# DIAGNijmegen/prostateMR_3D-CAD-csPCa

Hardware: AMD Instinct MI355X
Metric: train-step volumes/sec (whole job), M1 (20,160,160,3) (higher is better)
Workload: dtype bf16; 1 GPU; C3 M1 full hierarchical-probabilistic dense_skip+deep_supervision latents (3,2,1,0) (20,160,160,3); batch_per_gpu=2, global_batch=2, params=67254246, parallelism=dp1, hip_graph=True

## Files before the change

prostatemr_3d-cad-cspca_amd/csrc/conv_mfma.h:

```cpp
#pragma once
#include "common.h"
#include "gather.h"
#include "cdna4.h"

#define MF_MAX_TAPS 27
#define MF_MAX_CLASSES 8

struct MfmaP {
    const void* src[M1_MAX_SRC];
    int srcC[M1_MAX_SRC];
    int srcSeg[M1_MAX_SRC];
    int nsrc, CC, spt;
    int ID, IH, IW;
    void* out;
    int OC, OCn;
    int nout;
    void* outs[M1_MAX_SRC]; int outC[M1_MAX_SRC]; int outOff[M1_MAX_SRC + 1]; int outAcc[M1_MAX_SRC];
    int OD, OH, OW, N;
    const void* wp;
    const float* bias;
    const float* bias2; int bias_split;
    int mode, sd, sh, sw, pd, ph, pw;
    int nclasses;
    int cls_ntaps[MF_MAX_CLASSES], cls_first[MF_MAX_CLASSES], cls_kpad[MF_MAX_CLASSES];
    long long cls_woff[MF_MAX_CLASSES];
    signed char tdd[MF_MAX_TAPS], tdh[MF_MAX_TAPS], tdw[MF_MAX_TAPS];
    int tap_pk[MF_MAX_TAPS];
    int accumulate;
    int ksplit;
    float* acc32;
    long long slab_elems;
    int aligned;
    int korder;
    const void* ib_x;
    const float* ib_stats; const float* ib_gamma; const float* ib_beta; float ib_slope;
    int tps;
    float* stat_partial;
    int stat_tiles;
};

struct OutRef { void* base; int C, col, acc; };
__device__ __forceinline__ OutRef m1_out_ref(const MfmaP& p, int oc) {
    if (p.nout == 0) return OutRef{p.out, p.OC, oc, p.accumulate};
    int m = 0;
    while (m + 1 < p.nout && oc >= p.outOff[m + 1]) ++m;
    return OutRef{p.outs[m], p.outC[m], oc - p.outOff[m], p.outAcc[m]};
}

__device__ __forceinline__ float m1_bias_at(const MfmaP& p, int oc) {
    if (p.bias_split > 0 && oc >= p.bias_split) return p.bias2 ? p.bias2[oc - p.bias_split] : 0.f;
    return p.bias ? p.bias[oc] : 0.f;
}

template <typename T> struct MT;
template <> struct MT<bf16_t> { static constexpr int SEG = 8; };
template <> struct MT<float> { static constexpr int SEG = 4; };


bool m1_halo_conv_supported(const MfmaP& mp, int OCpad);
int m1_halo_conv_stat_parts(const MfmaP& mp, int OCpad);
int m1_halo_conv(const MfmaP& mp, int OCpad, hipStream_t st);

bool m1_pw_conv_supported(const MfmaP& mp, int OCpad, int BN);
int m1_pw_conv_stat_parts(const MfmaP& mp, int OCpad, int BN);
int m1_pw_conv(const MfmaP& mp, int OCpad, int BN, hipStream_t st);
```

prostatemr_3d-cad-cspca_amd/csrc/conv_mfma.hip:

```cpp
#include "common.h"
#include "gather.h"
#include "reduce.h"

#include "conv_mfma.h"
#include "conv_t3.h"
#include <stdlib.h>

template <typename T>
__device__ __forceinline__ uint4 load_partial_seg(const T* p, int n) {
    constexpr int SEG = MT<T>::SEG;
    union { uint4 v; T e[SEG]; } u;
    u.v = make_uint4(0, 0, 0, 0);
#pragma unroll
    for (int k = 0; k < SEG; ++k) if (k < n) u.e[k] = p[k];
    return u.v;
}

__device__ __forceinline__ unsigned lds_addr_of(const void* p) { return (unsigned)(unsigned long long)(lptr_t)p; }

template <typename T, int BM, int BN, int WM, int WN, int KC, bool GLDS, int KG = 1>
__global__ void __launch_bounds__(WM * WN * 64 * KG) conv_mfma_kernel(MfmaP p) {
#if defined(__HIP_DEVICE_COMPILE__)
    constexpr int NTHR = WM * WN * 64, NW = WM * WN;
    static_assert(KG == 1 || GLDS, "K groups: LDS-DMA path only");
    constexpr int SEG = MT<T>::SEG;
    constexpr int TM = BM / WM / 16, TN = BN / WN / 16;
    constexpr int A_BYTES = BM * 64, B_BYTES = BN * 64;
    constexpr int A_LD = BM * 4 / NTHR;
    constexpr int B_LD = (BN * 4 + NTHR - 1) / NTHR;
    static_assert((NW == 4 || NW == 8 || NW == 16) && (BM * 4) % NTHR == 0 && BN % 16 == 0, "tile config");

    extern __shared__ __attribute__((aligned(16))) unsigned char smem[];
    int4* rowinfo = reinterpret_cast<int4*>(smem);
    int* outrow = reinterpret_cast<int*>(rowinfo + BM);
    const T** s_src = reinterpret_cast<const T**>(outrow + BM);
    int* s_srcC = reinterpret_cast<int*>(s_src + M1_MAX_SRC);
    int* s_srcSeg = s_srcC + M1_MAX_SRC;
    int* s_tap = s_srcSeg + M1_MAX_SRC;
    int* s_tdl = s_tap + MF_MAX_TAPS;
    constexpr int TBL_BYTES = (BM * 20 + M1_MAX_SRC * 16 + 2 * MF_MAX_TAPS * 4 + 15) / 16 * 16;
    const int kg = KG > 1 ? __builtin_amdgcn_readfirstlane((int)threadIdx.x / NTHR) : 0;
    const int tid = KG > 1 ? (int)threadIdx.x - kg * NTHR : (int)threadIdx.x, lane = tid & 63, wave = tid >> 6;
    constexpr int GROUP_BYTES = 2 * KC * (A_BYTES + B_BYTES);
    unsigned char* A_s = smem + TBL_BYTES + kg * GROUP_BYTES;
    unsigned char* B_s = A_s + 2 * KC * A_BYTES;

    const int wm = wave / WN, wn = wave % WN;
    const int cls = blockIdx.y / p.ksplit, ksp = (blockIdx.y % p.ksplit) * KG + kg;
    const int oc0 = blockIdx.z * BN;

    int pdc = 0, phc = 0, pwc = 0, QD = p.OD, QH = p.OH, QW = p.OW;
    if (p.mode == 1) {
        pwc = cls % p.sw; phc = (cls / p.sw) % p.sh; pdc = cls / (p.sw * p.sh);
        QD = p.OD > pdc ? (p.OD - pdc + p.sd - 1) / p.sd : 0;
        QH = p.OH > phc ? (p.OH - phc + p.sh - 1) / p.sh : 0;
        QW = p.OW > pwc ? (p.OW - pwc + p.sw - 1) / p.sw : 0;
    }
    const long long QV = (long long)QD * QH * QW, Mtot = QV * p.N;
    const long long tile = (long long)(blockIdx.x & 7) * (gridDim.x >> 3) + (blockIdx.x >> 3);
    long long m0 = tile * BM, m_end = Mtot;
    if (p.tps > 0) {
        if (tile >= (long long)p.tps * p.N) return;
        const long long tn = tile / p.tps;
        m0 = tn * QV + (tile - tn * p.tps) * BM; m_end = (tn + 1) * QV;
    }
    if (m0 >= Mtot) return;

    for (int r = tid; r < BM; r += NTHR) {
        const long long m = m0 + r;
        int4 ri = make_int4(-1, 0, 0, 0); int orow = -1;
        if (m < m_end) {
            int n, qw, qh, qd;
            if (Mtot < (1ll << 31)) {
                const unsigned mm = (unsigned)m, qv = (unsigned)QV;
                n = (int)(mm / qv); const unsigned lin = mm - (unsigned)n * qv;
                const unsigned t1 = lin / (unsigned)QW; qw = (int)(lin - t1 * (unsigned)QW);
                qd = (int)(t1 / (unsigned)QH); qh = (int)(t1 - (unsigned)qd * (unsigned)QH);
            } else {
                n = (int)(m / QV); long long lin = m % QV;
                qw = (int)(lin % QW); lin /= QW; qh = (int)(lin % QH); qd = (int)(lin / QH);
            }
            if (p.mode == 0) {
                ri = make_int4(n, qd * p.sd - p.pd, qh * p.sh - p.ph, qw * p.sw - p.pw);
                orow = (int)m;
            } else {
                ri = make_int4(n, qd, qh, qw);
                orow = (int)((((long long)n * p.OD + qd * p.sd + pdc) * p.OH + qh * p.sh + phc) * p.OW + qw * p.sw + pwc);
            }
        }
        rowinfo[r] = ri; outrow[r] = orow;
    }
    if (tid < M1_MAX_SRC) { s_src[tid] = (const T*)p.src[tid]; s_srcC[tid] = p.srcC[tid]; s_srcSeg[tid] = p.srcSeg[tid]; }
    const int ntaps = p.cls_ntaps[cls], tfirst = p.cls_first[cls];
    if (tid < ntaps) {
        const int t = tfirst + tid;
        s_tap[tid] = ((int)p.tdd[t] & 0xff) | (((int)p.tdh[t] & 0xff) << 8) | (((int)p.tdw[t] & 0xff) << 16);
        s_tdl[tid] = ((int)p.tdd[t] * p.IH + (int)p.tdh[t]) * p.IW + (int)p.tdw[t];
    }
    __syncthreads();

    const int spt = p.spt;
    const int nseg = ntaps * spt;
    const int nchunks_all = (nseg + 3) >> 2;
    const int cps = (nchunks_all + p.ksplit * KG - 1) / (p.ksplit * KG);
    const int c_beg = ksp * cps;
    const int nchunks = (c_beg + cps <= nchunks_all ? cps : nchunks_all - c_beg);
    const int kpad = p.cls_kpad[cls];
    const T* wp = (const T*)p.wp + p.cls_woff[cls];

    f32x4_t acc[TM][TN];
#pragma unroll
    for (int i = 0; i < TM; ++i)
#pragma unroll
        for (int j = 0; j < TN; ++j) acc[i][j] = (f32x4_t){0.f, 0.f, 0.f, 0.f};

    uint4 ra[GLDS ? 1 : KC][GLDS ? 1 : A_LD], rb[GLDS ? 1 : KC][GLDS ? 1 : B_LD];
    const int lrow = tid >> 2;
    const int lseg = GLDS ? ((tid & 3) ^ ((-(tid >> 4)) & 3)) : (tid & 3);
    const int wave_u = __builtin_amdgcn_readfirstlane(wave);

    int st_tap = 0, st_s = 0, st_c = 0;
    const T* st_ptr[A_LD];
    auto st_set_tap = [&]() {
        const int tp = s_tap[st_tap];
        const int dd = (signed char)(tp & 0xff), dh = (signed char)((tp >> 8) & 0xff), dw = (signed char)((tp >> 16) & 0xff);
#pragma unroll
        for (int i = 0; i < A_LD; ++i) {
            const int4 ri = rowinfo[lrow + (NTHR / 4) * i];
            const int id = ri.y + dd, ih = ri.z + dh, iw = ri.w + dw;
            st_ptr[i] = nullptr;
            if (ri.x >= 0 && id >= 0 && id < p.ID && ih >= 0 && ih < p.IH && iw >= 0 && iw < p.IW) {
                const long long vox = (((long long)ri.x * p.ID + id) * p.IH + ih) * p.IW + iw;
                st_ptr[i] = s_src[st_s] + vox * s_srcC[st_s] + lseg * SEG;
            }
        }
    };
    constexpr unsigned OOB = 0x80000000u;
    unsigned b_vo[B_LD];
    unsigned rmask[A_LD]; int rvox[A_LD], rbyte[A_LD];
    int tap_db = 0;
    __amdgpu_buffer_rsrc_t rs_a = __builtin_amdgcn_make_buffer_rsrc((void*)p.src[0], 0, 0, 0x00020000);
    auto glds_set_member = [&]() {
        const int sC = __builtin_amdgcn_readfirstlane(s_srcC[st_s]);
#pragma unroll
        for (int i = 0; i < A_LD; ++i) rbyte[i] = (rvox[i] * sC + lseg * SEG) * (int)sizeof(T);
        rs_a = __builtin_amdgcn_make_buffer_rsrc((void*)p.src[__builtin_amdgcn_readfirstlane(st_s)], 0, 0x7fffffff, 0x00020000);
    };
    auto glds_set_tap = [&]() {
        tap_db = __builtin_amdgcn_readfirstlane(s_tdl[st_tap]) * __builtin_amdgcn_readfirstlane(s_srcC[st_s]) * (int)sizeof(T);
    };
    if constexpr (GLDS) {
        int4 ris[A_LD];
#pragma unroll
        for (int i = 0; i < A_LD; ++i) { ris[i] = rowinfo[lrow + (NTHR / 4) * i]; rmask[i] = 0; }
#pragma unroll 9
        for (int t = 0; t < ntaps; ++t) {
            const int tp = s_tap[t];
            const int dd = (signed char)(tp & 0xff), dh = (signed char)((tp >> 8) & 0xff), dw = (signed char)((tp >> 16) & 0xff);
#pragma unroll
            for (int i = 0; i < A_LD; ++i) {
                const bool ok = ris[i].x >= 0 && (unsigned)(ris[i].y + dd) < (unsigned)p.ID && (unsigned)(ris[i].z + dh) < (unsigned)p.IH &&
                                (unsigned)(ris[i].w + dw) < (unsigned)p.IW;
                rmask[i] |= (ok ? 1u : 0u) << t;
            }
        }
#pragma unroll
        for (int i = 0; i < A_LD; ++i) rvox[i] = ((ris[i].x * p.ID + ris[i].y) * p.IH + ris[i].z) * p.IW + ris[i].w;
    }
    if constexpr (GLDS) {
#pragma unroll
        for (int i = 0; i < B_LD; ++i) {
            const int e = tid + NTHR * i;
            b_vo[i] = (unsigned)(((oc0 + (e >> 2)) * kpad + lseg * SEG) * (int)sizeof(T));
        }
    }
    if (p.aligned && nchunks > 0) {
        const int cpt = spt >> 2;
        int c;
        if (p.korder == 2) { const int cg = c_beg / (2 * ntaps), rem = c_beg - cg * 2 * ntaps; st_tap = rem >> 1; c = (cg * 2 + (rem & 1)) * 4 * SEG; }
        else if (p.korder) { const int cg = c_beg / ntaps; st_tap = c_beg - cg * ntaps; c = cg * 4 * SEG; }
        else { st_tap = c_beg / cpt; c = (c_beg - st_tap * cpt) * 4 * SEG; }
        while (c >= s_srcC[st_s]) { c -= s_srcC[st_s]; ++st_s; }
        st_c = c;
        if constexpr (GLDS) { glds_set_member(); glds_set_tap(); } else st_set_tap();
    }

    auto prefetch_stage = [&](int sg) {
#pragma unroll
        for (int kc = 0; kc < KC; ++kc) {
            const int rel = sg * KC + kc;
            const int chunk = c_beg + rel;
            const bool live = rel < nchunks;
#pragma unroll
            for (int i = 0; i < B_LD; ++i) {
                const int e = tid + NTHR * i;
                uint4 v = make_uint4(0, 0, 0, 0);
                if (live && e < BN * 4)
                    v = *reinterpret_cast<const uint4*>(wp + (long long)(oc0 + (e >> 2)) * kpad + (long long)(chunk * 4 + (e & 3)) * SEG);
                rb[kc][i] = v;
            }
            if (!live) {
#pragma unroll
                for (int i = 0; i < A_LD; ++i) ra[kc][i] = make_uint4(0, 0, 0, 0);
            } else if (p.aligned) {
#pragma unroll
                for (int i = 0; i < A_LD; ++i)
                    ra[kc][i] = st_ptr[i] ? *reinterpret_cast<const uint4*>(st_ptr[i] + st_c) : make_uint4(0, 0, 0, 0);
                st_c += 4 * SEG;
                if (st_c >= s_srcC[st_s]) {
                    st_c = 0;
                    if (++st_s == p.nsrc) { st_s = 0; ++st_tap; }
                    if (st_tap < ntaps) st_set_tap();
                }
            } else {
                const int kseg = chunk * 4 + lseg;
                const T* sp = nullptr; int sC = 0, coff = 0, dd = 0, dh = 0, dw = 0;
                const bool kvalid = kseg < nseg;
                if (kvalid) {
                    const int tap_i = kseg / spt;
                    int cs = kseg - tap_i * spt, s = 0;
                    while (cs >= s_srcSeg[s]) { cs -= s_srcSeg[s]; ++s; }
                    sp = s_src[s]; sC = s_srcC[s]; coff = cs * SEG;
                    const int tp = s_tap[tap_i];
                    dd = (signed char)(tp & 0xff); dh = (signed char)((tp >> 8) & 0xff); dw = (signed char)((tp >> 16) & 0xff);
                }
#pragma unroll
                for (int i = 0; i < A_LD; ++i) {
                    const int4 ri = rowinfo[lrow + (NTHR / 4) * i];
                    uint4 v = make_uint4(0, 0, 0, 0);
                    const int id = ri.y + dd, ih = ri.z + dh, iw = ri.w + dw;
                    if (kvalid && coff < sC && ri.x >= 0 && id >= 0 && id < p.ID && ih >= 0 && ih < p.IH && iw >= 0 && iw < p.IW) {
                        const long long vox = (((long long)ri.x * p.ID + id) * p.IH + ih) * p.IW + iw;
                        if (sC % SEG == 0) v = *reinterpret_cast<const uint4*>(sp + vox * sC + coff);
                        else v = load_partial_seg<T>(sp + vox * sC + coff, sC - coff < SEG ? sC - coff : SEG);
                    }
                    ra[kc][i] = v;
                }
            }
        }
    };
    const __amdgpu_buffer_rsrc_t rs_b = __builtin_amdgcn_make_buffer_rsrc((void*)wp, 0, 0x7fffffff, 0x00020000);
    const __amdgpu_buffer_rsrc_t rs_0 = __builtin_amdgcn_make_buffer_rsrc((void*)wp, 0, 0, 0x00020000);
    auto issue_chunk = [&](int kc, int buf, int chunk, const __amdgpu_buffer_rsrc_t ra, const __amdgpu_buffer_rsrc_t rb) {
#pragma unroll
        for (int i = 0; i < B_LD; ++i)
            if ((NW * (i + 1)) * 64 <= BN * 4 || (wave_u + NW * i) * 64 < BN * 4)
                __builtin_amdgcn_raw_ptr_buffer_load_lds(rb, (lptr_t)(B_s + (buf * KC + kc) * B_BYTES + (wave_u + NW * i) * 1024), 16,
                                                         b_vo[i], chunk * 64, 0, 0);
#pragma unroll
        for (int i = 0; i < A_LD; ++i) {
            const unsigned vo = ((rmask[i] >> st_tap) & 1u) ? (unsigned)(rbyte[i] + tap_db) : OOB;
            __builtin_amdgcn_raw_ptr_buffer_load_lds(ra, (lptr_t)(A_s + (buf * KC + kc) * A_BYTES + (wave_u + NW * i) * 1024), 16,
                                                     vo, st_c * (int)sizeof(T), 0, 0);
        }
    };
    auto advance_chunk = [&]() {
        if (p.korder == 2) {
            if (((st_c / (4 * SEG)) & 1) == 0) st_c += 4 * SEG;
            else {
                st_c -= 4 * SEG;
                if (++st_tap == ntaps) {
                    st_tap = 0; st_c += 8 * SEG;
                    if (st_c >= s_srcC[st_s]) { st_c = 0; if (++st_s < p.nsrc) glds_set_member(); }
                }
                if (st_s < p.nsrc) glds_set_tap();
            }
        } else if (p.korder) {
            if (++st_tap == ntaps) {
                st_tap = 0; st_c += 4 * SEG;
                if (st_c >= s_srcC[st_s]) { st_c = 0; if (++st_s < p.nsrc) glds_set_member(); }
            }
            if (st_s < p.nsrc) glds_set_tap();
        } else {
            st_c += 4 * SEG;
            if (st_c >= s_srcC[st_s]) {
                st_c = 0;
                if (++st_s == p.nsrc) { st_s = 0; ++st_tap; }
                if (st_tap < ntaps) { glds_set_member(); glds_set_tap(); }
            }
        }
    };
    auto issue = [&](int sg, int buf) {
        const int rel0 = sg * KC;
        if (rel0 + KC <= nchunks) {
#pragma unroll
            for (int kc = 0; kc < KC; ++kc) { issue_chunk(kc, buf, c_beg + rel0 + kc, rs_a, rs_b); advance_chunk(); }
        } else {
#pragma unroll
            for (int kc = 0; kc < KC; ++kc) {
                const bool live = rel0 + kc < nchunks;
                issue_chunk(kc, buf, c_beg + rel0 + kc, live ? rs_a : rs_0, live ? rs_b : rs_0);
                if (live) advance_chunk();
            }
        }
    };
    auto stage = [&](int buf) {
#pragma unroll
        for (int kc = 0; kc < KC; ++kc) {
#pragma unroll
            for (int i = 0; i < A_LD; ++i) {
                const int row = lrow + (NTHR / 4) * i;
                *reinterpret_cast<uint4*>(A_s + (buf * KC + kc) * A_BYTES + row * 64 + m1_swz64(row, lseg) * 16) = ra[kc][i];
            }
#pragma unroll
            for (int i = 0; i < B_LD; ++i) {
                const int e = tid + NTHR * i;
                if (e < BN * 4) {
                    const int row = e >> 2;
                    *reinterpret_cast<uint4*>(B_s + (buf * KC + kc) * B_BYTES + row * 64 + m1_swz64(row, e & 3) * 16) = rb[kc][i];
                }
            }
        }
    };

    const int fr = lane & 15, fs = lane >> 4;
    const unsigned a_rd = lds_addr_of(A_s) + (wm * (BM / WM) + fr) * 64 + m1_swz64(fr, fs) * 16;
    const unsigned b_rd = lds_addr_of(B_s) + (wn * (BN / WN) + fr) * 64 + m1_swz64(fr, fs) * 16;
    const int nstages = KG > 1 ? (cps + KC - 1) / KC : (nchunks + KC - 1) / KC;
    if (nstages > 0) {
        if constexpr (GLDS) issue(0, 0);
        else { prefetch_stage(0); stage(0); }
    }
    __syncthreads();
    for (int it = 0; it < nstages; ++it) {
        const int buf = it & 1;
        if (it + 1 < nstages) { if constexpr (GLDS) issue(it + 1, buf ^ 1); else prefetch_stage(it + 1); }
        if constexpr (GLDS) {
            u32x4_t af[KC][TM], bfr[KC][TN];
            auto rd = [&](int kc) {
#pragma unroll
                for (int i = 0; i < TM; ++i) af[kc][i] = m1_lds_read128(a_rd + (buf * KC + kc) * A_BYTES + i * 1024);
#pragma unroll
                for (int j = 0; j < TN; ++j) bfr[kc][j] = m1_lds_read128(b_rd + (buf * KC + kc) * B_BYTES + j * 1024);
            };
            rd(0);
#pragma unroll
            for (int kc = 0; kc < KC; ++kc) {
                m1_lds_wait(af[kc][0]);
#pragma unroll
                for (int i = 1; i < TM; ++i) m1_lds_tie(af[kc][i]);
#pragma unroll
                for (int j = 0; j < TN; ++j) m1_lds_tie(bfr[kc][j]);
                if (kc + 1 < KC) rd(kc + 1);
                __builtin_amdgcn_sched_barrier(0);
#pragma unroll
                for (int i = 0; i < TM; ++i)
#pragma unroll
                    for (int j = 0; j < TN; ++j) {
                        if constexpr (sizeof(T) == 2) {
                            acc[i][j] = __builtin_amdgcn_mfma_f32_16x16x32_bf16(__builtin_bit_cast(bf16x8_t, af[kc][i]),
                                                                                __builtin_bit_cast(bf16x8_t, bfr[kc][j]), acc[i][j], 0, 0, 0);
                        } else {
#pragma unroll
                            for (int q = 0; q < 4; ++q)
                                acc[i][j] = __builtin_amdgcn_mfma_f32_16x16x4f32(__uint_as_float(af[kc][i][q]), __uint_as_float(bfr[kc][j][q]), acc[i][j], 0, 0, 0);
                        }
                    }
                if (kc + 1 < KC) __builtin_amdgcn_sched_barrier(0);
            }
        } else {
#pragma unroll
        for (int kc = 0; kc < KC; ++kc) {
            uint4 af[TM], bfr[TN];
#pragma unroll
            for (int i = 0; i < TM; ++i) {
                const int row = wm * (BM / WM) + i * 16 + fr;
                af[i] = *reinterpret_cast<const uint4*>(A_s + (buf * KC + kc) * A_BYTES + row * 64 + m1_swz64(row, fs) * 16);
            }
#pragma unroll
            for (int j = 0; j < TN; ++j) {
                const int row = wn * (BN / WN) + j * 16 + fr;
                bfr[j] = *reinterpret_cast<const uint4*>(B_s + (buf * KC + kc) * B_BYTES + row * 64 + m1_swz64(row, fs) * 16);
            }
#pragma unroll
            for (int i = 0; i < TM; ++i)
#pragma unroll
                for (int j = 0; j < TN; ++j) {
                    if constexpr (sizeof(T) == 2) {
                        acc[i][j] = __builtin_amdgcn_mfma_f32_16x16x32_bf16(__builtin_bit_cast(bf16x8_t, af[i]),
                                                                            __builtin_bit_cast(bf16x8_t, bfr[j]), acc[i][j], 0, 0, 0);
                    } else {
                        acc[i][j] = __builtin_amdgcn_mfma_f32_16x16x4f32(__uint_as_float(af[i].x), __uint_as_float(bfr[j].x), acc[i][j], 0, 0, 0);
                        acc[i][j] = __builtin_amdgcn_mfma_f32_16x16x4f32(__uint_as_float(af[i].y), __uint_as_float(bfr[j].y), acc[i][j], 0, 0, 0);
                        acc[i][j] = __builtin_amdgcn_mfma_f32_16x16x4f32(__uint_as_float(af[i].z), __uint_as_float(bfr[j].z), acc[i][j], 0, 0, 0);
                        acc[i][j] = __builtin_amdgcn_mfma_f32_16x16x4f32(__uint_as_float(af[i].w), __uint_as_float(bfr[j].w), acc[i][j], 0, 0, 0);
                    }
                }
        }
        }
        if constexpr (!GLDS) { if (it + 1 < nstages) stage(buf ^ 1); }
        __syncthreads();
    }

    if constexpr (KG > 1) {
        float* const xr = reinterpret_cast<float*>(smem + TBL_BYTES);
        if (kg > 0) {
            float* dst = xr + ((size_t)(kg - 1) * NTHR + tid) * (TM * TN * 4);
#pragma unroll
            for (int i = 0; i < TM; ++i)
#pragma unroll
                for (int j = 0; j < TN; ++j) *reinterpret_cast<f32x4_t*>(dst + (i * TN + j) * 4) = acc[i][j];
        }
        __syncthreads();
        if (kg > 0) return;
#pragma unroll
        for (int g = 1; g < KG; ++g) {
            const float* src = xr + ((size_t)(g - 1) * NTHR + tid) * (TM * TN * 4);
#pragma unroll
            for (int i = 0; i < TM; ++i)
#pragma unroll
                for (int j = 0; j < TN; ++j) acc[i][j] += *reinterpret_cast<const f32x4_t*>(src + (i * TN + j) * 4);
        }
        __syncthreads();
    }
    if (p.ksplit > 1) {
        float* slab = p.acc32 + (long long)ksp * p.slab_elems;
#pragma unroll
        for (int i = 0; i < TM; ++i)
#pragma unroll
            for (int j = 0; j < TN; ++j) {
                const int oc = oc0 + wn * (BN / WN) + j * 16 + fr;
#pragma unroll
                for (int r = 0; r < 4; ++r) {
                    const int orow = outrow[wm * (BM / WM) + i * 16 + fs * 4 + r];
                    if (orow >= 0 && oc < p.OCn) slab[(long long)orow * p.OC + oc] = acc[i][j][r];
                }
            }
        return;
    }
    constexpr int CP = BN + SEG;
    T* C_s = reinterpret_cast<T*>(A_s);
#pragma unroll
    for (int i = 0; i < TM; ++i)
#pragma unroll
        for (int j = 0; j < TN; ++j) {
            const int col = wn * (BN / WN) + j * 16 + fr;
            const float bv = (oc0 + col < p.OCn) ? m1_bias_at(p, oc0 + col) : 0.f;
#pragma unroll
            for (int r = 0; r < 4; ++r) {
                const int row = wm * (BM / WM) + i * 16 + fs * 4 + r;
                Act<T>::st(C_s + row * CP + col, acc[i][j][r] + bv);
            }
        }
    __syncthreads();
    if (p.stat_partial) {
        constexpr int EPI_BYTES = (int)((BM * CP * sizeof(T) + 15) / 16 * 16), PIPE_BYTES = 2 * KC * (A_BYTES + B_BYTES) * KG;
        float* red = reinterpret_cast<float*>(A_s + (PIPE_BYTES > EPI_BYTES ? PIPE_BYTES : EPI_BYTES));
        constexpr int G = NTHR / BN;
        const int col = tid % BN, rg = tid / BN;
        float s = 0.f, ss = 0.f;
        if (p.ib_x) {
            const int oc = oc0 + col < p.OCn ? oc0 + col : 0, n = (int)(m0 / QV);
            const float mean = p.ib_stats[((long long)n * p.OC + oc) * 2], rstd = p.ib_stats[((long long)n * p.OC + oc) * 2 + 1];
            const float gm = p.ib_gamma[oc], bt = p.ib_beta[oc];
            const T* xb = (const T*)p.ib_x + oc;
            constexpr int RPT = (BM + G - 1) / G;
            if constexpr (RPT > 32) {
                for (int row = rg; row < BM; row += G) {
                    const int orow = outrow[row];
                    if (orow >= 0) {
                        const float xh = (Act<T>::ld(xb + (long long)orow * p.OC) - mean) * rstd;
                        const float dy = Act<T>::ld(C_s + row * CP + col) * lrelu_g(gm * xh + bt, p.ib_slope);
                        s += dy; ss += dy * xh;
                    }
                }
            } else {
            float xv[RPT];
#pragma unroll
            for (int i = 0; i < RPT; ++i) {
                const int row = rg + i * G;
                const int orow = row < BM ? outrow[row] : -1;
                xv[i] = orow >= 0 ? Act<T>::ld(xb + (long long)orow * p.OC) : 0.f;
            }
#pragma unroll
            for (int i = 0; i < RPT; ++i) {
                const int row = rg + i * G;
                if (row < BM && outrow[row] >= 0) {
                    const float xh = (xv[i] - mean) * rstd;
                    const float dy = Act<T>::ld(C_s + row * CP + col) * lrelu_g(gm * xh + bt, p.ib_slope);
                    s += dy; ss += dy * xh;
                }
            }
            }
        } else
        for (int row = rg; row < BM; row += G) {
            if (outrow[row] >= 0) { const float v = Act<T>::ld(C_s + row * CP + col); s += v; ss += v * v; }
        }
        red[tid * 2] = s; red[tid * 2 + 1] = ss;
        __syncthreads();
        if (rg == 0 && oc0 + col < p.OCn) {
            for (int q = 1; q < G; ++q) { s += red[(q * BN + col) * 2]; ss += red[(q * BN + col) * 2 + 1]; }
            float* dst = p.stat_partial + ((tile * p.OC) + oc0 + col) * 2;
            dst[0] = s; dst[1] = ss;
        }
    }
    constexpr int SPR = BN / SEG;
    for (int e = tid; e < BM * SPR; e += NTHR) {
        const int row = e / SPR, cs = e % SPR;
        const int orow = outrow[row];
        const int oc = oc0 + cs * SEG;
        if (orow < 0 || oc >= p.OCn) continue;
        const OutRef o = m1_out_ref(p, oc);
        if (!o.base) continue;
        uint4 v = *reinterpret_cast<const uint4*>(C_s + row * CP + cs * SEG);
        T* dst = (T*)o.base + (long long)orow * o.C + o.col;
        if (o.C % SEG != 0 || (p.nout == 0 && oc + SEG > p.OCn)) {
            union { uint4 q; T e[SEG]; } ve; ve.q = v;
#pragma unroll
            for (int k = 0; k < SEG; ++k) {
                if (oc + k < p.OCn) {
                    float a = Act<T>::ld(&ve.e[k]);
                    if (o.acc) a += Act<T>::ld(dst + k);
                    Act<T>::st(dst + k, a);
                }
            }
            continue;
        }
        if (o.acc) {
            float a[SEG], b[SEG];
            VecIO<T, SEG>::ld(reinterpret_cast<const T*>(&v), a);
            VecIO<T, SEG>::ld(dst, b);
#pragma unroll
            for (int k = 0; k < SEG; ++k) a[k] += b[k];
            VecIO<T, SEG>::st(dst, a);
        } else {
            *reinterpret_cast<uint4*>(dst) = v;
        }
    }
#endif
}

template <typename T, int BM, int BN, int KC, int NTHR, int KG = 1>
static constexpr size_t mfma_smem_bytes() {
    size_t tbl = (BM * 20 + M1_MAX_SRC * 16 + 2 * MF_MAX_TAPS * 4 + 15) / 16 * 16;
    size_t pipe = (size_t)KC * (2 * BM * 64 + 2 * BN * 64) * KG;
    size_t epi = ((size_t)BM * (BN + MT<T>::SEG) * sizeof(T) + 15) / 16 * 16;
    return tbl + (pipe > epi ? pipe : epi) + NTHR * 2 * sizeof(float);
}

struct PackP {
    const float* w; long long wST, wSC, wSO; int oc_off, cc_off, OCn, OCpad, CC;
    const float* w2; long long w2ST, w2SC, w2SO; int oc_split, c_split;
    int nsrc, spt, SEG; int srcC[M1_MAX_SRC], srcSeg[M1_MAX_SRC];
    int nclasses; int cls_ntaps[MF_MAX_CLASSES], cls_first[MF_MAX_CLASSES], cls_kpad[MF_MAX_CLASSES];
    long long cls_woff[MF_MAX_CLASSES];
    unsigned char wtap[MF_MAX_TAPS];
    int korder;
};
__device__ __forceinline__ bool pack_seg_pos(const PackP& p, int cls, int kseg, int* nvalid, int* wtap, int* chan) {
    int tap_i, seg;
    if (p.korder == 2) {
        const int chunk = kseg >> 2, nt = p.cls_ntaps[cls], cg = chunk / (2 * nt), rem = chunk - cg * 2 * nt;
        tap_i = rem >> 1; seg = (cg * 2 + (rem & 1)) * 4 + (kseg & 3);
    } else if (p.korder) {
        const int chunk = kseg >> 2, nt = p.cls_ntaps[cls], cg = chunk / nt;
        tap_i = chunk - cg * nt; seg = cg * 4 + (kseg & 3);
    } else { tap_i = kseg / p.spt; seg = kseg - tap_i * p.spt; }
    int c = 0, s = 0;
    while (s < p.nsrc && seg >= p.srcSeg[s]) { seg -= p.srcSeg[s]; c += p.srcC[s]; ++s; }
    if (s >= p.nsrc || tap_i >= p.cls_ntaps[cls]) { *nvalid = 0; return false; }
    const int rem = p.srcC[s] - seg * p.SEG;
    *nvalid = rem < p.SEG ? rem : p.SEG;
    *chan = c + seg * p.SEG;
    *wtap = p.wtap[p.cls_first[cls] + tap_i];
    return true;
}
#define M1_PACK_JOB_BYTES 512
#define M1_PACK_MAGIC 0x4d315031u
struct PackJob { PackP p; void* out; int dtype; unsigned magic; };
static_assert(sizeof(PackJob) <= M1_PACK_JOB_BYTES, "pack job record");

template <typename T>
__device__ __forceinline__ void pack_class_elems(const PackP& p, int cls, T* __restrict__ out, long long first, long long stride) {
    constexpr int SEG = MT<T>::SEG;
    const int kpad = p.cls_kpad[cls], nks = kpad / SEG;
    const bool oc_fast = p.wSO == 1;
    const int ocg = p.OCpad >> 4, ksg = (nks + 3) >> 2;
    const long long tot = oc_fast ? (long long)ocg * ksg * 64 : (long long)p.OCpad * nks;
    for (long long u = first; u < tot; u += stride) {
        int oc, kseg;
        if (oc_fast) {
            const long long grp = u >> 6; const int l = (int)(u & 63);
            oc = (int)(grp % ocg) * 16 + (l & 15); kseg = (int)(grp / ocg) * 4 + (l >> 4);
            if (kseg >= nks) continue;
        } else { oc = (int)(u / nks); kseg = (int)(u % nks); }
        int nvalid, wtap = 0, c = 0;
        pack_seg_pos(p, cls, kseg, &nvalid, &wtap, &c);
// ... 103 lines not shown
    }
    __device__ void vec(int n, long long v, int c0, float (*acc)[kVec]) const {
        const long long row = (long long)n * V + v, i = row * OC + c0;
        float a[kVec];
#pragma unroll
        for (int e = 0; e < kVec; ++e) {
            const int oc = c0 + e;
            a[e] = (bias_split > 0 && oc >= bias_split) ? (bias2 ? bias2[oc - bias_split] : 0.f) : (bias ? bias[oc] : 0.f);
        }
        for (int k = 0; k < ksplit; ++k) {
            const float* sp = acc32 + (long long)k * slab + i;
#pragma unroll
            for (int q = 0; q < kVec; q += 4) {
                const float4 t = *reinterpret_cast<const float4*>(sp + q);
                a[q] += t.x; a[q + 1] += t.y; a[q + 2] += t.z; a[q + 3] += t.w;
            }
        }
        T* dst = out + i;
        if (fo.nout > 0) {
            int m = 0;
            while (m + 1 < fo.nout && c0 >= fo.outOff[m + 1]) ++m;
            dst = (T*)fo.outs[m] + row * fo.outC[m] + (c0 - fo.outOff[m]);
        }
        VecIO<T, kVec>::st(dst, a);
        float xv[kVec];
        if (ib_x) VecIO<T, kVec>::ld(ib_x + i, xv);
#pragma unroll
        for (int e = 0; e < kVec; ++e) {
            float r = a[e];
            if constexpr (sizeof(T) == 2) r = bf2f(f2bf(r));
            if (ib_x) {
                const int c = c0 + e;
                const float xh = (xv[e] - ib_stats[((long long)n * OC + c) * 2]) * ib_stats[((long long)n * OC + c) * 2 + 1];
                const float dy = r * lrelu_g(ib_gamma[c] * xh + ib_beta[c], ib_slope);
                acc[0][e] += dy; acc[1][e] += dy * xh;
            } else { acc[0][e] += r; acc[1][e] += r * r; }
        }
    }
};

static inline int seg_of(int dtype) { return dtype == M1_BF16 ? 8 : 4; }
static inline int pick_bn(int ocn) { return ocn > 64 ? 128 : (ocn > 32 ? 64 : (ocn > 16 ? 32 : 16)); }
struct Plan { int BN, BM, ksplit; };
static inline bool want_bn160(const GatherSpec& g) {
    int en = M1_CFG("M1_BN160", 1);
    return en && g.dtype == M1_BF16 && g.w2 && g.oc_split > 0 && g.mode == 0 && g.OC % 160 == 0 && g.OC <= 320;
}
static inline Plan make_plan(int ocn, long long maxM, int ncls, int min_nchunks, bool bn160 = false) {
    Plan pl; pl.BN = bn160 ? 160 : pick_bn(ocn);
    const int ntile = (ocn + pl.BN - 1) / pl.BN;
    pl.BM = (bn160 || cdiv_ll(maxM, 128) * ncls * ntile >= 256) ? 128 : 64;
    const long long blocks = cdiv_ll(maxM, pl.BM) * ncls * ntile;
    pl.ksplit = 1;
    {
        int t128 = M1_CFG("M1_PLAN128", 768);
        const long long b128 = cdiv_ll(maxM, 128) * ncls * ntile;
        if (t128 > 0 && pl.BN == 128 && b128 >= 100 && b128 < t128 && min_nchunks >= 200) {
            pl.BM = 128;
            long long want = cdiv_ll(t128, b128), cap = min_nchunks / 64;
            pl.ksplit = (int)(want < cap ? want : cap);
            if (pl.ksplit < 1) pl.ksplit = 1;
            return pl;
        }
    }
    if (blocks < 256 && min_nchunks >= 16) {
        long long want = cdiv_ll(512, blocks), cap = min_nchunks / 8;
        pl.ksplit = (int)(want < cap ? want : cap);
        if (pl.ksplit < 1) pl.ksplit = 1;
        if (pl.ksplit > 32) pl.ksplit = 32;
    }
    return pl;
}
static inline long long spec_maxM(const GatherSpec& g) {
    if (g.mode == 0) return (long long)g.N * g.OD * g.OH * g.OW;
    return (long long)g.N * ((g.OD + g.sd - 1) / g.sd) * ((g.OH + g.sh - 1) / g.sh) * ((g.OW + g.sw - 1) / g.sw);
}
static inline int spec_ncls(const GatherSpec& g) { return g.mode == 1 ? g.sd * g.sh * g.sw : 1; }

bool m1_mfma_supported(const GatherSpec& g) {
    if (g.kd * g.kh * g.kw > MF_MAX_TAPS) return false;
    if (g.mode == 1 && g.sd * g.sh * g.sw > MF_MAX_CLASSES) return false;
    return true;
}

static inline int spec_spt(const GatherSpec& g, int SEG) {
    int s = 0; for (int i = 0; i < g.nsrc; ++i) s += (g.srcC[i] + SEG - 1) / SEG; return s;
}
static void build_classes(const GatherSpec& g, int CC, int SEG, int OCpad, MfmaP* mp, PackP* pp, long long* total_elems) {
    const int ncls = g.mode == 1 ? g.sd * g.sh * g.sw : 1;
    int t = 0; long long woff = 0;
    for (int c = 0; c < ncls; ++c) {
        const int pwc = g.mode == 1 ? c % g.sw : 0, phc = g.mode == 1 ? (c / g.sw) % g.sh : 0, pdc = g.mode == 1 ? c / (g.sw * g.sh) : 0;
        const int first = t;
        for (int a = 0; a < g.kd; ++a) {
            int od;
            if (g.mode == 0) od = a - 0; else { int v = pdc + g.pd - a; if (v % g.sd) continue; od = v / g.sd; }
            for (int b = 0; b < g.kh; ++b) {
                int oh;
                if (g.mode == 0) oh = b; else { int v = phc + g.ph - b; if (v % g.sh) continue; oh = v / g.sh; }
                for (int e = 0; e < g.kw; ++e) {
                    int ow;
                    if (g.mode == 0) ow = e; else { int v = pwc + g.pw - e; if (v % g.sw) continue; ow = v / g.sw; }
                    if (mp) { mp->tdd[t] = (signed char)od; mp->tdh[t] = (signed char)oh; mp->tdw[t] = (signed char)ow; }
                    if (pp) pp->wtap[t] = (unsigned char)((a * g.kh + b) * g.kw + e);
                    ++t;
                }
            }
        }
        const int nt = t - first;
        const int nseg = nt * spec_spt(g, SEG);
        const int kpad = ((nseg + 3) / 4) * 4 * SEG;
        if (mp) { mp->cls_ntaps[c] = nt; mp->cls_first[c] = first; mp->cls_kpad[c] = kpad; mp->cls_woff[c] = woff; }
        if (pp) { pp->cls_ntaps[c] = nt; pp->cls_first[c] = first; pp->cls_kpad[c] = kpad; pp->cls_woff[c] = woff; }
        woff += (long long)OCpad * kpad;
    }
    if (mp) mp->nclasses = ncls;
    if (pp) pp->nclasses = ncls;
    *total_elems = woff;
}

static inline int min_class_chunks(const GatherSpec& g, int CC, int SEG) {
    MfmaP tmp{}; long long tot = 0;
    build_classes(g, CC, SEG, 16, &tmp, nullptr, &tot);
    int mn = 1 << 30;
    for (int c = 0; c < tmp.nclasses; ++c) { int n = tmp.cls_kpad[c] / (4 * SEG); if (n < mn) mn = n; }
    return mn;
}
static inline size_t out_elems(const GatherSpec& g) { return (size_t)g.N * g.OD * g.OH * g.OW * g.OC; }

size_t m1_mfma_ws_bytes(const GatherSpec& g) {
    const int SEG = seg_of(g.dtype);
    int CC = 0; for (int i = 0; i < g.nsrc; ++i) CC += g.srcC[i];
    size_t best = 0;
    const bool maybe160 = g.dtype == M1_BF16 && g.mode == 0 && g.OC % 160 == 0 && g.OC <= 320;
    int t3bn = 0, t3ks = 1;
    const bool t3 = m1_ct3_plan(g, &t3bn, &t3ks);
    for (int v = 0; v < 3; ++v) {
        if ((v == 1 && !maybe160) || (v == 2 && !t3)) continue;
        Plan pl = make_plan(g.OC, spec_maxM(g), spec_ncls(g), min_class_chunks(g, CC, SEG), v == 1);
        if (v == 2) { pl.BN = t3bn; pl.BM = 256; pl.ksplit = t3ks; }
        const int BN = pl.BN, OCpad = (g.OC + BN - 1) / BN * BN;
        long long tot = 0;
        build_classes(g, CC, SEG, OCpad, nullptr, nullptr, &tot);
        size_t bytes = ((size_t)tot * (g.dtype == M1_BF16 ? 2 : 4) + 255) / 256 * 256;
        if (pl.ksplit > 1) bytes += out_elems(g) * sizeof(float) * pl.ksplit;
        if (bytes > best) best = bytes;
    }
    return best + 256 + M1_PACK_JOB_BYTES;
}

template <typename T, int BM, int BN, int WM, int WN, int KC>
static int launch_cfg_kc(const MfmaP& mp, long long maxM, int OCpad, hipStream_t st) {
    dim3 grid((unsigned)(cdiv_ll(cdiv_ll(maxM, BM), 8) * 8), mp.nclasses * mp.ksplit, OCpad / BN);
    const size_t smem = mfma_smem_bytes<T, BM, BN, KC, WM * WN * 64>();
    auto kern = mp.aligned ? conv_mfma_kernel<T, BM, BN, WM, WN, KC, true> : conv_mfma_kernel<T, BM, BN, WM, WN, KC, false>;
    if (smem > 48 * 1024 && m1_allow_dynamic_lds((const void*)kern, (int)smem) != M1_OK) return M1_ERR_LAUNCH;
    m1_note_kernel("conv_mfma:%dx%d:w%d:ks%d", BM, BN, WM * WN, mp.ksplit);
    hipLaunchKernelGGL(kern, grid, dim3(WM * WN * 64), smem, st, mp);
    return m1_check_launch();
}

template <typename T, int BM, int BN, int WM, int WN, int KG>
static int launch_cfg_kg(const MfmaP& mp, long long maxM, int OCpad, hipStream_t st) {
    constexpr size_t smem = mfma_smem_bytes<T, BM, BN, 2, WM * WN * 64, KG>();
    if constexpr (sizeof(T) != 2 || smem > 160 * 1024 - 256 || WM * WN * 64 * KG > 1024) return M1_ERR_UNSUPPORTED;
    else {
        dim3 grid((unsigned)(cdiv_ll(cdiv_ll(maxM, BM), 8) * 8), mp.nclasses * mp.ksplit, OCpad / BN);
        if (m1_allow_dynamic_lds((const void*)conv_mfma_kernel<T, BM, BN, WM, WN, 2, true, KG>, (int)smem) != M1_OK) return M1_ERR_LAUNCH;
        m1_note_kernel("conv_mfma:%dx%d:w%d:ks%d:kg%d", BM, BN, WM * WN, mp.ksplit, KG);
        hipLaunchKernelGGL((conv_mfma_kernel<T, BM, BN, WM, WN, 2, true, KG>), grid, dim3(WM * WN * 64 * KG), smem, st, mp);
        return m1_check_launch();
    }
}
static inline int mfma_kg_max(int BM, int BN, int nthr) {
    const int group = 2 * 2 * (BM + BN) * 64;
    int k = (150 * 1024) / group; if (k > 1024 / nthr) k = 1024 / nthr; if (k > 4) k = 4;
    return k >= 2 ? k : 0;
}

template <typename T, int BM, int BN, int WM, int WN>
static int launch_cfg(const MfmaP& mp, long long maxM, int OCpad, hipStream_t st, int kg = 1) {
    if (kg == 2) return launch_cfg_kg<T, BM, BN, WM, WN, 2>(mp, maxM, OCpad, st);
    if (kg == 3) return launch_cfg_kg<T, BM, BN, WM, WN, 3>(mp, maxM, OCpad, st);
    if (kg == 4) return launch_cfg_kg<T, BM, BN, WM, WN, 4>(mp, maxM, OCpad, st);
    int minchunks = 1 << 30;
    for (int c = 0; c < mp.nclasses; ++c) { const int n = mp.cls_kpad[c] / (4 * MT<T>::SEG) / mp.ksplit; if (n < minchunks) minchunks = n; }
    return minchunks >= 6 ? launch_cfg_kc<T, BM, BN, WM, WN, 2>(mp, maxM, OCpad, st)
                          : launch_cfg_kc<T, BM, BN, WM, WN, 1>(mp, maxM, OCpad, st);
}

template <typename T>
static int run_mfma(const GatherSpec& g, void* ws, int ws_packed, hipStream_t st) {
    constexpr int SEG = MT<T>::SEG;
    MfmaP mp{}; PackP pp{};
    int CC = 0;
    for (int i = 0; i < M1_MAX_SRC; ++i) {
        mp.src[i] = i < g.nsrc ? g.src[i] : nullptr; mp.srcC[i] = i < g.nsrc ? g.srcC[i] : (1 << 30);
        mp.srcSeg[i] = i < g.nsrc ? (g.srcC[i] + SEG - 1) / SEG : (1 << 30);
        pp.srcC[i] = i < g.nsrc ? g.srcC[i] : 0; pp.srcSeg[i] = i < g.nsrc ? (g.srcC[i] + SEG - 1) / SEG : 0;
        if (i < g.nsrc) CC += g.srcC[i];
    }
    mp.nsrc = g.nsrc; mp.CC = CC; mp.spt = spec_spt(g, SEG);
    pp.nsrc = g.nsrc; pp.spt = mp.spt; pp.SEG = SEG; mp.ID = g.ID; mp.IH = g.IH; mp.IW = g.IW; mp.out = g.out; mp.OC = g.OC; mp.OCn = g.OC;
    void* panel = reinterpret_cast<unsigned char*>(ws) + M1_PACK_JOB_BYTES;
    mp.OD = g.OD; mp.OH = g.OH; mp.OW = g.OW; mp.N = g.N; mp.wp = panel; mp.bias = g.bias; mp.mode = g.mode;
// ... 188 lines not shown
```

Measured before the change: 92.81 volumes/s.

## Add persistent tile-loop variant of MFMA conv kernel with double-buffered row tables

Adds a PERSIST template variant of the conv MFMA kernel that loops over several M tiles per block. It hoists the B offsets out of the loop and decodes the next tile's row table into a second LDS buffer during the epilogue. When LDS space allows, the epilogue staging is placed after the first pipeline stage. The host launches it with a grid capped at occupancy times CU count, by default only for BN=32 aligned, ksplit=1 convs with more than 256 tiles. The aim is to cut block launch and prologue overhead and overlap epilogue work with the next tile's setup, at the cost of more LDS and a possible loss in occupancy.

```diff
diff --git a/prostatemr_3d-cad-cspca_amd/csrc/conv_mfma.h b/prostatemr_3d-cad-cspca_amd/csrc/conv_mfma.h
--- a/prostatemr_3d-cad-cspca_amd/csrc/conv_mfma.h
+++ b/prostatemr_3d-cad-cspca_amd/csrc/conv_mfma.h
@@ -35,6 +35,7 @@
     const void* ib_x;
     const float* ib_stats; const float* ib_gamma; const float* ib_beta; float ib_slope;
     int tps;
+    int ptiles;
     float* stat_partial;
     int stat_tiles;
 };
diff --git a/prostatemr_3d-cad-cspca_amd/csrc/conv_mfma.hip b/prostatemr_3d-cad-cspca_amd/csrc/conv_mfma.hip
--- a/prostatemr_3d-cad-cspca_amd/csrc/conv_mfma.hip
+++ b/prostatemr_3d-cad-cspca_amd/csrc/conv_mfma.hip
@@ -18,11 +18,12 @@
 
 __device__ __forceinline__ unsigned lds_addr_of(const void* p) { return (unsigned)(unsigned long long)(lptr_t)p; }
 
-template <typename T, int BM, int BN, int WM, int WN, int KC, bool GLDS, int KG = 1>
+template <typename T, int BM, int BN, int WM, int WN, int KC, bool GLDS, int KG = 1, bool PERSIST = false>
 __global__ void __launch_bounds__(WM * WN * 64 * KG) conv_mfma_kernel(MfmaP p) {
 #if defined(__HIP_DEVICE_COMPILE__)
     constexpr int NTHR = WM * WN * 64, NW = WM * WN;
     static_assert(KG == 1 || GLDS, "K groups: LDS-DMA path only");
+    static_assert(!PERSIST || (GLDS && KG == 1), "tile loop: LDS-DMA path, one K group");
     constexpr int SEG = MT<T>::SEG;
     constexpr int TM = BM / WM / 16, TN = BN / WN / 16;
     constexpr int A_BYTES = BM * 64, B_BYTES = BN * 64;
@@ -31,19 +32,24 @@
     static_assert((NW == 4 || NW == 8 || NW == 16) && (BM * 4) % NTHR == 0 && BN % 16 == 0, "tile config");
 
     extern __shared__ __attribute__((aligned(16))) unsigned char smem[];
-    int4* rowinfo = reinterpret_cast<int4*>(smem);
-    int* outrow = reinterpret_cast<int*>(rowinfo + BM);
-    const T** s_src = reinterpret_cast<const T**>(outrow + BM);
+    constexpr int NTBL = PERSIST ? 2 : 1;
+    int4* const rowinfo0 = reinterpret_cast<int4*>(smem);
+    int* const outrow0 = reinterpret_cast<int*>(rowinfo0 + NTBL * BM);
+    int4* rowinfo = rowinfo0;
+    int* outrow = outrow0;
+    const T** s_src = reinterpret_cast<const T**>(outrow0 + NTBL * BM);
     int* s_srcC = reinterpret_cast<int*>(s_src + M1_MAX_SRC);
     int* s_srcSeg = s_srcC + M1_MAX_SRC;
     int* s_tap = s_srcSeg + M1_MAX_SRC;
     int* s_tdl = s_tap + MF_MAX_TAPS;
-    constexpr int TBL_BYTES = (BM * 20 + M1_MAX_SRC * 16 + 2 * MF_MAX_TAPS * 4 + 15) / 16 * 16;
+    constexpr int TBL_BYTES = (NTBL * BM * 20 + M1_MAX_SRC * 16 + 2 * MF_MAX_TAPS * 4 + 15) / 16 * 16;
     const int kg = KG > 1 ? __builtin_amdgcn_readfirstlane((int)threadIdx.x / NTHR) : 0;
     const int tid = KG > 1 ? (int)threadIdx.x - kg * NTHR : (int)threadIdx.x, lane = tid & 63, wave = tid >> 6;
     constexpr int GROUP_BYTES = 2 * KC * (A_BYTES + B_BYTES);
+    constexpr int STAGE_BYTES = KC * (A_BYTES + B_BYTES);
+    constexpr int A_BUF = PERSIST ? STAGE_BYTES : KC * A_BYTES, B_BUF = PERSIST ? STAGE_BYTES : KC * B_BYTES;
     unsigned char* A_s = smem + TBL_BYTES + kg * GROUP_BYTES;
-    unsigned char* B_s = A_s + 2 * KC * A_BYTES;
+    unsigned char* B_s = A_s + (PERSIST ? KC * A_BYTES : 2 * KC * A_BYTES);
 
     const int wm = wave / WN, wn = wave % WN;
     const int cls = blockIdx.y / p.ksplit, ksp = (blockIdx.y % p.ksplit) * KG + kg;
@@ -57,21 +63,28 @@
         QW = p.OW > pwc ? (p.OW - pwc + p.sw - 1) / p.sw : 0;
     }
     const long long QV = (long long)QD * QH * QW, Mtot = QV * p.N;
-    const long long tile = (long long)(blockIdx.x & 7) * (gridDim.x >> 3) + (blockIdx.x >> 3);
-    long long m0 = tile * BM, m_end = Mtot;
-    if (p.tps > 0) {
-        if (tile >= (long long)p.tps * p.N) return;
-        const long long tn = tile / p.tps;
-        m0 = tn * QV + (tile - tn * p.tps) * BM; m_end = (tn + 1) * QV;
-    }
-    if (m0 >= Mtot) return;
-
+    const int xtiles = PERSIST ? p.ptiles : (int)(gridDim.x >> 3);
+    int xt = (int)(blockIdx.x >> 3);
+    long long tile = (long long)(blockIdx.x & 7) * xtiles + xt;
+    auto tile_rows = [&](long long t, long long& m0_, long long& m_end_) -> bool {
+        m0_ = t * BM; m_end_ = Mtot;
+        if (p.tps > 0) {
+            if (t >= (long long)p.tps * p.N) return false;
+            const long long tn = t / p.tps;
+            m0_ = tn * QV + (t - tn * p.tps) * BM; m_end_ = (tn + 1) * QV;
+        }
+        return m0_ < Mtot;
+    };
+    long long m0, m_end;
+    if (!tile_rows(tile, m0, m_end)) return;
+
+    auto decode_rows = [&](long long m0, long long m_end, int4* rowinfo, int* outrow) {
     for (int r = tid; r < BM; r += NTHR) {
         const long long m = m0 + r;
         int4 ri = make_int4(-1, 0, 0, 0); int orow = -1;
         if (m < m_end) {
             int n, qw, qh, qd;
-            if (Mtot < (1ll << 31)) {
+            if (PERSIST || Mtot < (1ll << 31)) {
                 const unsigned mm = (unsigned)m, qv = (unsigned)QV;
                 n = (int)(mm / qv); const unsigned lin = mm - (unsigned)n * qv;
                 const unsigned t1 = lin / (unsigned)QW; qw = (int)(lin - t1 * (unsigned)QW);
@@ -90,6 +103,8 @@
         }
         rowinfo[r] = ri; outrow[r] = orow;
     }
+    };
+    decode_rows(m0, m_end, rowinfo, outrow);
     if (tid < M1_MAX_SRC) { s_src[tid] = (const T*)p.src[tid]; s_srcC[tid] = p.srcC[tid]; s_srcSeg[tid] = p.srcSeg[tid]; }
     const int ntaps = p.cls_ntaps[cls], tfirst = p.cls_first[cls];
     if (tid < ntaps) {
@@ -108,16 +123,26 @@
     const int kpad = p.cls_kpad[cls];
     const T* wp = (const T*)p.wp + p.cls_woff[cls];
 
-    f32x4_t acc[TM][TN];
-#pragma unroll
-    for (int i = 0; i < TM; ++i)
-#pragma unroll
-        for (int j = 0; j < TN; ++j) acc[i][j] = (f32x4_t){0.f, 0.f, 0.f, 0.f};
-
-    uint4 ra[GLDS ? 1 : KC][GLDS ? 1 : A_LD], rb[GLDS ? 1 : KC][GLDS ? 1 : B_LD];
     const int lrow = tid >> 2;
     const int lseg = GLDS ? ((tid & 3) ^ ((-(tid >> 4)) & 3)) : (tid & 3);
     const int wave_u = __builtin_amdgcn_readfirstlane(wave);
+    unsigned b_vo[B_LD];
+    if constexpr (GLDS) {
+#pragma unroll
+        for (int i = 0; i < B_LD; ++i) {
+            const int e = tid + NTHR * i;
+            b_vo[i] = (unsigned)(((oc0 + (e >> 2)) * kpad + lseg * SEG) * (int)sizeof(T));
+        }
+    }
+
+    for (int tb = 0;;) {
+    f32x4_t acc[TM][TN];
+#pragma unroll
+    for (int i = 0; i < TM; ++i)
+#pragma unroll
+        for (int j = 0; j < TN; ++j) acc[i][j] = (f32x4_t){0.f, 0.f, 0.f, 0.f};
+
+    uint4 ra[GLDS ? 1 : KC][GLDS ? 1 : A_LD], rb[GLDS ? 1 : KC][GLDS ? 1 : B_LD];
 
     int st_tap = 0, st_s = 0, st_c = 0;
     const T* st_ptr[A_LD];
@@ -136,7 +161,6 @@
         }
     };
     constexpr unsigned OOB = 0x80000000u;
-    unsigned b_vo[B_LD];
     unsigned rmask[A_LD]; int rvox[A_LD], rbyte[A_LD];
     int tap_db = 0;
     __amdgpu_buffer_rsrc_t rs_a = __builtin_amdgcn_make_buffer_rsrc((void*)p.src[0], 0, 0, 0x00020000);
@@ -166,13 +190,6 @@
         }
 #pragma unroll
         for (int i = 0; i < A_LD; ++i) rvox[i] = ((ris[i].x * p.ID + ris[i].y) * p.IH + ris[i].z) * p.IW + ris[i].w;
-    }
-    if constexpr (GLDS) {
-#pragma unroll
-        for (int i = 0; i < B_LD; ++i) {
-            const int e = tid + NTHR * i;
-            b_vo[i] = (unsigned)(((oc0 + (e >> 2)) * kpad + lseg * SEG) * (int)sizeof(T));
-        }
     }
     if (p.aligned && nchunks > 0) {
         const int cpt = spt >> 2;
@@ -245,12 +262,12 @@
 #pragma unroll
         for (int i = 0; i < B_LD; ++i)
             if ((NW * (i + 1)) * 64 <= BN * 4 || (wave_u + NW * i) * 64 < BN * 4)
-                __builtin_amdgcn_raw_ptr_buffer_load_lds(rb, (lptr_t)(B_s + (buf * KC + kc) * B_BYTES + (wave_u + NW * i) * 1024), 16,
+                __builtin_amdgcn_raw_ptr_buffer_load_lds(rb, (lptr_t)(B_s + buf * B_BUF + kc * B_BYTES + (wave_u + NW * i) * 1024), 16,
                                                          b_vo[i], chunk * 64, 0, 0);
 #pragma unroll
         for (int i = 0; i < A_LD; ++i) {
             const unsigned vo = ((rmask[i] >> st_tap) & 1u) ? (unsigned)(rbyte[i] + tap_db) : OOB;
-            __builtin_amdgcn_raw_ptr_buffer_load_lds(ra, (lptr_t)(A_s + (buf * KC + kc) * A_BYTES + (wave_u + NW * i) * 1024), 16,
+            __builtin_amdgcn_raw_ptr_buffer_load_lds(ra, (lptr_t)(A_s + buf * A_BUF + kc * A_BYTES + (wave_u + NW * i) * 1024), 16,
                                                      vo, st_c * (int)sizeof(T), 0, 0);
         }
     };
@@ -300,14 +317,14 @@
 #pragma unroll
             for (int i = 0; i < A_LD; ++i) {
                 const int row = lrow + (NTHR / 4) * i;
-                *reinterpret_cast<uint4*>(A_s + (buf * KC + kc) * A_BYTES + row * 64 + m1_swz64(row, lseg) * 16) = ra[kc][i];
+                *reinterpret_cast<uint4*>(A_s + buf * A_BUF + kc * A_BYTES + row * 64 + m1_swz64(row, lseg) * 16) = ra[kc][i];
             }
 #pragma unroll
             for (int i = 0; i < B_LD; ++i) {
                 const int e = tid + NTHR * i;
                 if (e < BN * 4) {
                     const int row = e >> 2;
-                    *reinterpret_cast<uint4*>(B_s + (buf * KC + kc) * B_BYTES + row * 64 + m1_swz64(row, e & 3) * 16) = rb[kc][i];
+                    *reinterpret_cast<uint4*>(B_s + buf * B_BUF + kc * B_BYTES + row * 64 + m1_swz64(row, e & 3) * 16) = rb[kc][i];
                 }
             }
         }
@@ -329,9 +346,9 @@
             u32x4_t af[KC][TM], bfr[KC][TN];
             auto rd = [&](int kc) {
 #pragma unroll
-                for (int i = 0; i < TM; ++i) af[kc][i] = m1_lds_read128(a_rd + (buf * KC + kc) * A_BYTES + i * 1024);
-#pragma unroll
-                for (int j = 0; j < TN; ++j) bfr[kc][j] = m1_lds_read128(b_rd + (buf * KC + kc) * B_BYTES + j * 1024);
+                for (int i = 0; i < TM; ++i) af[kc][i] = m1_lds_read128(a_rd + buf * A_BUF + kc * A_BYTES + i * 1024);
+#pragma unroll
+                for (int j = 0; j < TN; ++j) bfr[kc][j] = m1_lds_read128(b_rd + buf * B_BUF + kc * B_BYTES + j * 1024);
             };
             rd(0);
 #pragma unroll
@@ -365,12 +382,12 @@
 #pragma unroll
             for (int i = 0; i < TM; ++i) {
                 const int row = wm * (BM / WM) + i * 16 + fr;
-                af[i] = *reinterpret_cast<const uint4*>(A_s + (buf * KC + kc) * A_BYTES + row * 64 + m1_swz64(row, fs) * 16);
+                af[i] = *reinterpret_cast<const uint4*>(A_s + buf * A_BUF + kc * A_BYTES + row * 64 + m1_swz64(row, fs) * 16);
             }
 #pragma unroll
             for (int j = 0; j < TN; ++j) {
                 const int row = wn * (BN / WN) + j * 16 + fr;
-                bfr[j] = *reinterpret_cast<const uint4*>(B_s + (buf * KC + kc) * B_BYTES + row * 64 + m1_swz64(row, fs) * 16);
+                bfr[j] = *reinterpret_cast<const uint4*>(B_s + buf * B_BUF + kc * B_BYTES + row * 64 + m1_swz64(row, fs) * 16);
             }
 #pragma unroll
             for (int i = 0; i < TM; ++i)
@@ -428,26 +445,37 @@
             }
         return;
     }
+    int etid = tid;
+    if constexpr (PERSIST) asm volatile("" : "+v"(etid));
+    const int efr = etid & 15, efs = (etid & 63) >> 4, ewm = (etid >> 6) / WN, ewn = (etid >> 6) % WN;
     constexpr int CP = BN + SEG;
-    T* C_s = reinterpret_cast<T*>(A_s);
+    constexpr int EPI_BYTES = (int)((BM * CP * sizeof(T) + 15) / 16 * 16), PIPE_BYTES = 2 * KC * (A_BYTES + B_BYTES) * KG;
+    constexpr bool EPI_FREE = PERSIST && STAGE_BYTES + EPI_BYTES <= PIPE_BYTES;
+    T* C_s = reinterpret_cast<T*>(A_s + (EPI_FREE ? STAGE_BYTES : 0));
 #pragma unroll
     for (int i = 0; i < TM; ++i)
 #pragma unroll
         for (int j = 0; j < TN; ++j) {
-            const int col = wn * (BN / WN) + j * 16 + fr;
+            const int col = ewn * (BN / WN) + j * 16 + efr;
             const float bv = (oc0 + col < p.OCn) ? m1_bias_at(p, oc0 + col) : 0.f;
 #pragma unroll
             for (int r = 0; r < 4; ++r) {
-                const int row = wm * (BM / WM) + i * 16 + fs * 4 + r;
+                const int row = ewm * (BM / WM) + i * 16 + efs * 4 + r;
                 Act<T>::st(C_s + row * CP + col, acc[i][j][r] + bv);
             }
         }
+    long long nx_tile = 0, nx_m0 = 0, nx_end = 0; bool nx = false;
+    if constexpr (PERSIST) {
+        const int nb = (int)(gridDim.x >> 3);
+        nx_tile = tile + nb;
+        nx = xt + nb < xtiles && tile_rows(nx_tile, nx_m0, nx_end);
+        if (nx) decode_rows(nx_m0, nx_end, rowinfo0 + (tb ^ 1) * BM, outrow0 + (tb ^ 1) * BM);
+    }
     __syncthreads();
     if (p.stat_partial) {
-        constexpr int EPI_BYTES = (int)((BM * CP * sizeof(T) + 15) / 16 * 16), PIPE_BYTES = 2 * KC * (A_BYTES + B_BYTES) * KG;
         float* red = reinterpret_cast<float*>(A_s + (PIPE_BYTES > EPI_BYTES ? PIPE_BYTES : EPI_BYTES));
         constexpr int G = NTHR / BN;
-        const int col = tid % BN, rg = tid / BN;
+        const int col = etid % BN, rg = etid / BN;
         float s = 0.f, ss = 0.f;
         if (p.ib_x) {
             const int oc = oc0 + col < p.OCn ? oc0 + col : 0, n = (int)(m0 / QV);
@@ -486,7 +514,7 @@
         for (int row = rg; row < BM; row += G) {
             if (outrow[row] >= 0) { const float v = Act<T>::ld(C_s + row * CP + col); s += v; ss += v * v; }
         }
-        red[tid * 2] = s; red[tid * 2 + 1] = ss;
+        red[etid * 2] = s; red[etid * 2 + 1] = ss;
         __syncthreads();
         if (rg == 0 && oc0 + col < p.OCn) {
             for (int q = 1; q < G; ++q) { s += red[(q * BN + col) * 2]; ss += red[(q * BN + col) * 2 + 1]; }
@@ -495,7 +523,7 @@
         }
     }
     constexpr int SPR = BN / SEG;
-    for (int e = tid; e < BM * SPR; e += NTHR) {
+    for (int e = etid; e < BM * SPR; e += NTHR) {
         const int row = e / SPR, cs = e % SPR;
         const int orow = outrow[row];
         const int oc = oc0 + cs * SEG;
@@ -527,12 +555,20 @@
             *reinterpret_cast<uint4*>(dst) = v;
         }
     }
+    if constexpr (!PERSIST) return;
+    else {
+        if (!nx) return;
+        if constexpr (!EPI_FREE) __syncthreads();
+        tb ^= 1; rowinfo = rowinfo0 + tb * BM; outrow = outrow0 + tb * BM;
+        xt += (int)(gridDim.x >> 3); tile = nx_tile; m0 = nx_m0; m_end = nx_end;
+    }
+    }
 #endif
 }
 
-template <typename T, int BM, int BN, int KC, int NTHR, int KG = 1>
+template <typename T, int BM, int BN, int KC, int NTHR, int KG = 1, bool PERSIST = false>
 static constexpr size_t mfma_smem_bytes() {
-    size_t tbl = (BM * 20 + M1_MAX_SRC * 16 + 2 * MF_MAX_TAPS * 4 + 15) / 16 * 16;
+    size_t tbl = ((PERSIST ? 2 : 1) * BM * 20 + M1_MAX_SRC * 16 + 2 * MF_MAX_TAPS * 4 + 15) / 16 * 16;
     size_t pipe = (size_t)KC * (2 * BM * 64 + 2 * BN * 64) * KG;
     size_t epi = ((size_t)BM * (BN + MT<T>::SEG) * sizeof(T) + 15) / 16 * 16;
     return tbl + (pipe > epi ? pipe : epi) + NTHR * 2 * sizeof(float);
@@ -742,6 +778,7 @@
     pl.BM = (bn160 || cdiv_ll(maxM, 128) * ncls * ntile >= 256) ? 128 : 64;
     const long long blocks = cdiv_ll(maxM, pl.BM) * ncls * ntile;
     pl.ksplit = 1;
+    if (M1_CFG("M1_MFMA_PERSIST_BLOCKS", 0) > 0) { pl.BM = 128; return pl; }
     {
         int t128 = M1_CFG("M1_PLAN128", 768);
         const long long b128 = cdiv_ll(maxM, 128) * ncls * ntile;
@@ -839,8 +876,65 @@
     return best + 256 + M1_PACK_JOB_BYTES;
 }
 
+template <typename K>
+static int mfma_blocks_per_cu(K kern, int nthr, size_t smem) {
+    int nb = 0;
+    return hipOccupancyMaxActiveBlocksPerMultiprocessor(&nb, kern, nthr, smem) == hipSuccess ? nb : 0;
+}
+static int mfma_cu_count() {
+    static const int ncu = []() {
+        int dev = 0, n = 0;
+        if (hipGetDevice(&dev) != hipSuccess || hipDeviceGetAttribute(&n, hipDeviceAttributeMultiprocessorCount, dev) != hipSuccess) n = 0;
+        return n;
+    }();
+    return ncu;
+}
+
+template <typename T, int BM, int BN, int WM, int WN, int KC>
+static int launch_persistent(const MfmaP& mp_in, long long maxM, int OCpad, hipStream_t st, bool* done) {
+    *done = false;
+    if constexpr (BM != 128) return M1_OK;
+    else {
+        const int en = M1_CFG("M1_MFMA_PERSIST", 1);
+        if (!mp_in.aligned || mp_in.ksplit != 1 || !en) return M1_OK;
+        constexpr int NTHR = WM * WN * 64;
+        if (maxM >= (1ll << 31)) return M1_OK;
+        const long long tiles8 = cdiv_ll(cdiv_ll(maxM, BM), 8) * 8;
+        auto kern = conv_mfma_kernel<T, BM, BN, WM, WN, KC, true, 1, true>;
+        constexpr size_t smem = mfma_smem_bytes<T, BM, BN, KC, NTHR, 1, true>();
+        const int forced = M1_CFG("M1_MFMA_PERSIST_BLOCKS", 0);
+        long long cap = forced;
+        if (forced <= 0) {
+            if (BN != 32 && en < 2) return M1_OK;
+            if (tiles8 <= 256) return M1_OK;
+            static int per_cu = -1;
+            if (per_cu < 0) {
+                auto kern1 = conv_mfma_kernel<T, BM, BN, WM, WN, KC, true>;
+                constexpr size_t smem1 = mfma_smem_bytes<T, BM, BN, KC, NTHR>();
+                if (smem > 48 * 1024 && m1_allow_dynamic_lds((const void*)kern, (int)smem) != M1_OK) return M1_ERR_LAUNCH;
+                if (smem1 > 48 * 1024 && m1_allow_dynamic_lds((const void*)kern1, (int)smem1) != M1_OK) return M1_ERR_LAUNCH;
+                const int a = mfma_blocks_per_cu(kern, NTHR, smem), b = mfma_blocks_per_cu(kern1, NTHR, smem1);
+                per_cu = (a > 0 && a >= b) ? a : 0;
+            }
+            cap = (long long)per_cu * mfma_cu_count();
+        }
+        cap = cap / 8 * 8;
+        if (cap < 8 || tiles8 <= cap) return M1_OK;
+        if (smem > 48 * 1024 && m1_allow_dynamic_lds((const void*)kern, (int)smem) != M1_OK) return M1_ERR_LAUNCH;
+        MfmaP mp = mp_in;
+        mp.ptiles = (int)(tiles8 >> 3);
+        dim3 grid((unsigned)cap, mp.nclasses, OCpad / BN);
+        if (forced > 0) m1_note_kernel("conv_mfma:%dx%d:w%d:ks%d:pt%d", BM, BN, WM * WN, mp.ksplit, (int)cap);
+        else m1_note_kernel("conv_mfma:%dx%d:w%d:ks%d", BM, BN, WM * WN, mp.ksplit);
+        hipLaunchKernelGGL(kern, grid, dim3(NTHR), smem, st, mp);
+        *done = true;
+        return m1_check_launch();
+    }
+}
+
 template <typename T, int BM, int BN, int WM, int WN, int KC>
 static int launch_cfg_kc(const MfmaP& mp, long long maxM, int OCpad, hipStream_t st) {
+    { bool done = false; const int rc = launch_persistent<T, BM, BN, WM, WN, KC>(mp, maxM, OCpad, st, &done); if (rc || done) return rc; }
     dim3 grid((unsigned)(cdiv_ll(cdiv_ll(maxM, BM), 8) * 8), mp.nclasses * mp.ksplit, OCpad / BN);
     const size_t smem = mfma_smem_bytes<T, BM, BN, KC, WM * WN * 64>();
     auto kern = mp.aligned ? conv_mfma_kernel<T, BM, BN, WM, WN, KC, true> : conv_mfma_kernel<T, BM, BN, WM, WN, KC, false>;
```

Measured after the change: 92.81 volumes/s, median of 2. No clear change (-0.0%).
